# kehanxuuu/vspg-pbrt-v4

Hardware: AMD Instinct MI355X
Metric: Mpaths/sec on 1920x1080 homogeneous fog; relMSE vs CPU ref at equal spp (higher is better)
Workload: dtype f32; 1 GPU; fog-box 1920x1080, guidedvolpathvspg vspguiding=true (primary-ray VSP; App. F options), 1 spp per step per GPU, independent sampler seed 0, maxdepth 5

## Files before the change

### vspg-pbrt-v4_amd/csrc/vspg_capi.hip

```cpp
#include <hip/hip_runtime.h>
#include <dlfcn.h>

#include <cmath>
#include <cstdio>
#include <cstdlib>
#include <cstring>
#include <string>
#include <type_traits>
#include <vector>
#include <algorithm>

#include "vspg_path.h"
#include "vspg_wg_kernel.h"
#include "vspg_guided_wg.h"
#include "vspg_wg3.h"
#include "vspg_trace.h"
#include "vspg_wavefront.h"
#include "vspg_wf_launch.h"
#include "vspg_film_error.h"
#include "vspg_film_resolve.h"
#include "vspg_kernel_choice.h"
#ifdef VSPG_SINGLE_TU
#include "vspg_wf_grid.hip"
#include "vspg_wf_nvdb.hip"
// ... 1807 lines not shown
    return lb;
}
static void build(const VspgScene &sc, const VspgIntegratorParams &prm, DScene *D) {
    DLightSampler *ls = &D->lsamp;
    std::memset(ls, 0, sizeof *ls);
    const int n_all = D->n_lights + D->n_inf;
    for (int i = 0; i < kMaxLights; ++i) ls->bit_trail[i] = 0xffffffffu;
    for (int i = 0; i < VSPG_MAX_QUADS; ++i) ls->light_of_quad[i] = -1;
    for (int i = 0; i < D->n_lights; ++i) ls->light_of_quad[D->light_quads[i]] = i;
    ls->mode = n_all > 1 ? prm.lightsampler : VSPG_LIGHTSAMPLER_UNIFORM;
    lbvh_item_t items[LBVH_MAX_LIGHTS];
    int n_items = 0;
    v3 amin = V3(INFINITY, INFINITY, INFINITY), amax = V3(-INFINITY, -INFINITY, -INFINITY);
    for (int i = 0; i < n_all; ++i) {
        if (i >= D->n_lights) { ls->inf_light[ls->n_inf++] = i; continue; }
        const int qi = D->light_quads[i];
        lightbounds_t lb = quad_light_bounds(D->quads[qi], sc.quads[qi].reverse_orientation);
        if (lb.phi > 0) {
            items[n_items].light = i; items[n_items].lb = lb; n_items++;
            amin = v_min3(amin, lb.bmin); amax = v_max3(amax, lb.bmax);
        }
    }
    if (n_items > 0) { lightbounds_t root; lbvh_build(ls, items, 0, n_items, 0, 0, amin, amax, &root); }
    if (n_all > 0) {
        float pdf[3], power[LBVH_MAX_LIGHTS], acc0 = 0.f;
        for (int i = 0; i < 3; ++i) {
            float up = 0.5f + (float)i / 3;
            if (up > 1) up -= 1;
            float lambda = 538 - 138.888889f * atanhf(0.85691062f - 1.82750197f * up);
            pdf[i] = lambda < 360 || lambda > 830 ? 0.f : 0.0039398042f / sqr(coshf(0.0072f * (lambda - 538)));
        }
        for (int i = 0; i < n_all; ++i) {
            float L[3], k;
            if (i < D->n_lights) {
                const DQuad &q = D->quads[D->light_quads[i]];
                for (int c = 0; c < 3; ++c) L[c] = q.Le[c];
                k = PI_F * (q.two_sided ? 2 : 1) * q.area;
            } else {
                const int j = i - D->n_lights;
                for (int c = 0; c < 3; ++c) L[c] = D->inf_L[j][c];
                k = D->inf_type[j] == VSPG_LIGHT_DISTANT ? PI_F * sqr(D->scene_radius) : 4 * PI_F * PI_F * sqr(D->scene_radius);
            }
            float s = 0.f;
            for (int c = 0; c < 3; ++c) s += pdf[c] != 0 ? (k * L[c]) / pdf[c] : 0.f;
            power[i] = s / 3;
            acc0 += power[i];
        }
        if (acc0 == 0.f) for (int i = 0; i < n_all; ++i) power[i] = 1.f;
        double sum = 0.;
        for (int i = 0; i < n_all; ++i) sum += power[i];
        const float fsum = (float)sum;
        ls->n_alias = n_all;
        struct { float pHat; int index; } under[LBVH_MAX_LIGHTS], over[LBVH_MAX_LIGHTS];
        int nu = 0, no = 0;
        for (int i = 0; i < n_all; ++i) {
            ls->alias_p[i] = power[i] / fsum;
            float pHat = ls->alias_p[i] * n_all;
            if (pHat < 1) { under[nu].pHat = pHat; under[nu].index = i; nu++; } else { over[no].pHat = pHat; over[no].index = i; no++; }
        }
        while (nu > 0 && no > 0) {
            float upH = under[nu - 1].pHat, ovH = over[no - 1].pHat;
            int ui = under[nu - 1].index, oi = over[no - 1].index;
            nu--; no--;
            ls->alias_q[ui] = upH; ls->alias_i[ui] = oi;
            float pExcess = upH + ovH - 1;
            if (pExcess < 1) { under[nu].pHat = pExcess; under[nu].index = oi; nu++; } else { over[no].pHat = pExcess; over[no].index = oi; no++; }
        }
        while (no > 0) { no--; ls->alias_q[over[no].index] = 1; ls->alias_i[over[no].index] = -1; }
        while (nu > 0) { nu--; ls->alias_q[under[nu].index] = 1; ls->alias_i[under[nu].index] = -1; }
    }
}
}

static bool derive_triangle(const float *p9, const float *kd, int id, DTri *T, const int32_t *flags = nullptr);
static int32_t surf_flags_of(int material, int medium_interface) {
    const int b = medium_interface & (VSPG_IFACE_INSIDE | VSPG_IFACE_OUTSIDE);
    const int iface = (b == VSPG_IFACE_INSIDE || b == VSPG_IFACE_OUTSIDE) ? b : 0;
    return (material == VSPG_MATERIAL_INTERFACE ? SURF_INTERFACE : 0) | (iface << SURF_IFACE_SHIFT);
}
static void build_dscene(const VspgScene &sc, const VspgIntegratorParams &prm, const VspgRenderConfig &cfg, DScene *D) {
    using namespace hostmath;
    memset(D, 0, sizeof *D);
    D->n_quads = sc.n_quads;
    for (int i = 0; i < sc.n_quads; ++i) {
        const VspgQuad &in = sc.quads[i];
        DQuad &q = D->quads[i];
        H3 p00 = ld(in.p00), e1 = ld(in.e1), e2 = ld(in.e2);
        H3 p10 = add(p00, e1), p01 = add(p00, e2), p11 = add(p10, e2);
        stv(q.p00, p00); stv(q.p10, p10); stv(q.p01, p01); stv(q.p11, p11); stv(q.e1, e1); stv(q.e2, e2);
        H3 c = crossv(e1, e2);
        q.area = std::sqrt(len2v(c));
        H3 n = normv(c);
        if (in.reverse_orientation) n = H3{-n.x, -n.y, -n.z};
        stv(q.n, n);
        stv(q.dpdu_n, normv(e1));
        const float eps = 0x1p-24f;
        float g6 = (6 * eps) / (1 - 6 * eps);
        H3 s = add(add(absv(p00), absv(p01)), add(absv(p10), absv(p11)));
        stv(q.perr, H3{s.x * g6, s.y * g6, s.z * g6});
        q.inv_l1 = 1.f / len2v(e1);
        q.inv_l2 = 1.f / len2v(e2);
        bool lobes = false, light = false;
        for (int k = 0; k < 3; ++k) {
            float kd = in.Kd[k];
            kd = kd < 0 ? 0 : (kd > 1 ? 1 : kd);
            q.Kd[k] = kd;
            q.Le[k] = in.Le[k];
            lobes = lobes || kd != 0;
            light = light || in.Le[k] != 0;
        }
        q.two_sided = in.two_sided;
        q.is_light = light;
        q.has_lobes = lobes;
        q.flags = surf_flags_of(in.material, in.medium_interface);
        auto single_axis = [](const float *v) {
            int nz = 0, ax = -1;
            for (int k = 0; k < 3; ++k)
                if (v[k] != 0) { nz++; ax = k; }
            return nz == 1 ? ax : -1;
        };
        int an = single_axis(q.n), a1 = single_axis(q.e1), a2 = single_axis(q.e2);
        IsectRec &rec = D->irec[i];
        memset(&rec, 0, sizeof rec);
        if (an >= 0 && a1 >= 0 && a2 >= 0 && an != a1 && an != a2 && a1 != a2 && std::fabs(q.n[an]) == 1.0f) {
            rec.kind = 1;
            rec.axes = an | (a1 << 2) | (a2 << 4);
            rec.f[0] = q.n[an]; rec.f[1] = q.p00[an]; rec.f[2] = q.p00[a1]; rec.f[3] = q.p00[a2];
            rec.f[4] = q.e1[a1]; rec.f[5] = q.e2[a2]; rec.f[6] = q.inv_l1; rec.f[7] = q.inv_l2;
        } else {
            rec.kind = 0;
            for (int k = 0; k < 3; ++k) { rec.f[k] = q.n[k]; rec.f[3 + k] = q.p00[k]; rec.f[6 + k] = q.e1[k]; rec.f[9 + k] = q.e2[k]; }
            rec.f[12] = q.inv_l1; rec.f[13] = q.inv_l2;
        }
        if (light) D->light_quads[D->n_lights++] = i;
    }
    D->n_inf = sc.n_infinite_lights;
    for (int i = 0; i < sc.n_infinite_lights && i < VSPG_MAX_INFINITE_LIGHTS; ++i) {
        D->inf_type[i] = sc.infinite_lights[i].type;
        for (int k = 0; k < 3; ++k) { D->inf_L[i][k] = sc.infinite_lights[i].L[k]; D->inf_w[i][k] = sc.infinite_lights[i].w_light[k]; }
    }
    {
        float lo[3] = {kInf, kInf, kInf}, hi[3] = {-kInf, -kInf, -kInf};
        auto grow = [&](const float *q) { for (int k = 0; k < 3; ++k) { lo[k] = q[k] < lo[k] ? q[k] : lo[k]; hi[k] = q[k] > hi[k] ? q[k] : hi[k]; } };
        for (int i = 0; i < D->n_quads; ++i) { grow(D->quads[i].p00); grow(D->quads[i].p10); grow(D->quads[i].p01); grow(D->quads[i].p11); }
        for (int i = 0; i < sc.n_triangles && sc.tri_p; ++i) {
            DTri T;
            if (derive_triangle(sc.tri_p + 9 * (size_t)i, nullptr, i, &T)) { grow(T.p0); grow(T.p1); grow(T.p2); }
        }
        for (int i = 0; i < sc.n_spheres; ++i) {
            const float *m = sc.spheres[i].render_from_object, rr = sc.spheres[i].radius;
            for (int c = 0; c < 8; ++c) {
                const float x = (c & 1) ? rr : -rr, y = (c & 2) ? rr : -rr, z = (c & 4) ? rr : -rr;
                float q[3];
                for (int k = 0; k < 3; ++k) {
                    volatile float a = m[4 * k] * x;
                    volatile float b = m[4 * k + 1] * y;
                    volatile float c2 = m[4 * k + 2] * z;
                    volatile float sum = a + b;
                    sum = sum + c2;
                    sum = sum + m[4 * k + 3];
                    q[k] = sum;
                }
                grow(q);
            }
        }
        D->scene_radius = 0.f;
        if (lo[0] <= hi[0]) {
            volatile float cx = (lo[0] + hi[0]) / 2, cy = (lo[1] + hi[1]) / 2, cz = (lo[2] + hi[2]) / 2;
            volatile float dx = cx - hi[0], dy = cy - hi[1], dz = cz - hi[2];
            volatile float l2 = dx * dx;
            l2 = l2 + dy * dy;
            l2 = l2 + dz * dz;
            D->scene_radius = std::sqrt(l2);
        }
    }
    D->n_spheres = sc.n_spheres;
    for (int i = 0; i < sc.n_spheres; ++i) {
        const VspgSphere &in = sc.spheres[i];
        DSphere &sp = D->spheres[i];
        for (int k = 0; k < 12; ++k) { sp.m[k] = in.render_from_object[k]; sp.mi[k] = in.object_from_render[k]; }
        sp.radius = in.radius;
        const float *m = in.render_from_object;
        const float minor12 = dop(m[5], m[10], m[6], m[9]), minor02 = dop(m[4], m[10], m[6], m[8]), minor01 = dop(m[4], m[9], m[5], m[8]);
        const bool swaps = std::fmaf(m[2], minor01, dop(m[0], minor12, m[1], minor02)) < 0;
        sp.flip = (in.reverse_orientation ? 1 : 0) ^ (swaps ? 1 : 0);
        auto clamp1 = [](float v) { return v < -1.f ? -1.f : (v > 1.f ? 1.f : v); };
        sp.thetaZMin = std::acos(clamp1(-in.radius / in.radius));
        sp.thetaZMax = std::acos(clamp1(in.radius / in.radius));
        {
            volatile float rad = 3.14159265358979323846f / 180;
            rad = rad * 360.f;
            sp.phiMax = rad;
        }
        bool lobes = false;
        for (int k = 0; k < 3; ++k) {
            float kd = in.Kd[k];
            kd = kd < 0 ? 0 : (kd > 1 ? 1 : kd);
            sp.Kd[k] = kd;
            lobes = lobes || kd != 0;
        }
        sp.has_lobes = lobes;
        sp.flags = surf_flags_of(in.material, in.medium_interface);
    }
    D->camera_in_medium = sc.medium.type != VSPG_MEDIUM_NONE && !sc.camera_outside_medium;
    D->has_boundaries = sc.camera_outside_medium != 0;
    for (int i = 0; i < D->n_quads; ++i) D->has_boundaries |= D->quads[i].flags != 0;
    for (int i = 0; i < D->n_spheres; ++i) D->has_boundaries |= D->spheres[i].flags != 0;
    for (int i = 0; i < sc.n_triangles && sc.tri_flags; ++i)
        D->has_boundaries |= surf_flags_of(sc.tri_flags[i] & VSPG_TRI_INTERFACE, sc.tri_flags[i] >> VSPG_TRI_IFACE_SHIFT) != 0;
    D->cam = sc.camera;
    D->medium_type = sc.medium.type;
    for (int k = 0; k < 3; ++k) {
        D->sigma_a[k] = sc.medium.sigma_a[k];
        D->sigma_s[k] = sc.medium.sigma_s[k];
        {
            volatile float st = D->sigma_s[k] + D->sigma_a[k];
// ... 2049 lines not shown
```

### vspg-pbrt-v4_amd/csrc/vspg_device.h

```cpp
#pragma once
#include <hip/hip_runtime.h>
#include <stdint.h>

#include "../../include/vspg.h"
#include "vspg_arith.h"
#include "vspg_libm.h"

#define VDEV __device__ __forceinline__
#ifdef VSPG_WF_DEBUG
__device__ unsigned int g_dbg_err[8];
#define VSPG_DBG_CHECK(cond, bit) do { if (!(cond)) atomicOr(&g_dbg_err[0], 1u << (bit)); } while (0)
#else
#define VSPG_DBG_CHECK(cond, bit)
#endif
#ifdef VSPG_NOINLINE_LEAVES
#define VLEAF __device__ __attribute__((noinline))
#else
#define VLEAF __device__ __forceinline__
#endif

VSPG_NS_BEGIN

#ifdef VSPG_PROFILE
enum { PS_INTERSECT = 0, PS_HASHRNG, PS_DIST_GUIDED, PS_DIST_PLAIN, PS_SURF_PRE, PS_NEE, PS_NEE_TR, PS_VOL_SAMPLE,
// ... 343 lines not shown
    *cosTheta = ct;
    *sinTheta = safe_sqrt(1 - sqr(ct));
    return 2 * kPi * u1;
}
VDEV V3 hg_post(V3 wo, float g, float sinTheta, float cosTheta, float sinPhi, float cosPhi, float *pdf) {
    g = clampf(g, (float)-.99, (float).99);
    Frame f;
    f.z = wo;
    coordinate_system(wo, &f.x, &f.y);
    V3 local = V3{clampf(sinTheta, -1, 1) * cosPhi, clampf(sinTheta, -1, 1) * sinPhi, clampf(cosTheta, -1, 1)};
    *pdf = henyey_greenstein(cosTheta, g);
    return f.from_local(local);
}
VDEV V3 sample_henyey_greenstein(V3 wo, float g, float u0, float u1, float *pdf) {
    float st, ct;
    float phi = hg_pre(g, u0, u1, &st, &ct);
    return hg_post(wo, g, st, ct, sinf_(phi), cosf_(phi), pdf);
}
VDEV float cos_hemi_pre(float u0, float u1, float *r, bool *degenerate) {
    float ox = 2 * u0 - 1, oy = 2 * u1 - 1;
    *degenerate = (ox == 0 && oy == 0);
    const bool xmajor = __builtin_fabsf(ox) > __builtin_fabsf(oy);
    const float q = (xmajor ? oy : ox) / (xmajor ? ox : oy);
    *r = xmajor ? ox : oy;
    const float t = kPiOver4 * q;
    return xmajor ? t : kPiOver2 - t;
}
VDEV V3 cos_hemi_post(float r, bool degenerate, float sinT, float cosT) {
    float dx = degenerate ? 0.f : r * cosT;
    float dy = degenerate ? 0.f : r * sinT;
    float z = safe_sqrt(1 - sqr(dx) - sqr(dy));
    return V3{dx, dy, z};
}
VDEV V3 sample_cosine_hemisphere(float u0, float u1) {
    float r;
    bool deg;
    float theta = cos_hemi_pre(u0, u1, &r, &deg);
    return cos_hemi_post(r, deg, sinf_(theta), cosf_(theta));
}

struct P3i {
    V3 lo, hi;
    VDEV V3 mid() const { return V3{(lo.x + hi.x) / 2, (lo.y + hi.y) / 2, (lo.z + hi.z) / 2}; }
    VDEV V3 err() const { return V3{(hi.x - lo.x) / 2, (hi.y - lo.y) / 2, (hi.z - lo.z) / 2}; }
};
VDEV P3i p3i_exact(V3 p) { return P3i{p, p}; }
VDEV void interval_ve(float v, float e, float *lo, float *hi) {
    float l = next_float_down(v - e), h = next_float_up(v + e);
    *lo = e == 0 ? v : l;
    *hi = e == 0 ? v : h;
}
VDEV P3i p3i_from_err(V3 p, V3 e) {
    P3i r;
    interval_ve(p.x, e.x, &r.lo.x, &r.hi.x);
    interval_ve(p.y, e.y, &r.lo.y, &r.hi.y);
    interval_ve(p.z, e.z, &r.lo.z, &r.hi.z);
    return r;
}
VDEV float offset_axis(float po, float off) {
    const uint32_t ui = f2b(po), os = f2b(off) & 0x80000000u;
    uint32_t r = ui + ((uint32_t)((int32_t)(ui ^ os) >> 31) | 1u);
    r = (ui << 1) == 0u ? (os | 1u) : r;
    const bool keep = !__builtin_islessgreater(off, 0.f) || (ui ^ os) == 0x7f800000u;
    return b2f(keep ? ui : r);
}
VDEV V3 offset_ray_origin(P3i pi, V3 n, V3 w) {
    float d = dot(vabs(n), pi.err());
    V3 offset = n * d;
    if (dot(w, n) < 0) offset = -offset;
    V3 po = pi.mid() + offset;
    return V3{offset_axis(po.x, offset.x), offset_axis(po.y, offset.y), offset_axis(po.z, offset.z)};
}

#define VSPG_GLOBAL_AS __attribute__((address_space(1)))
struct DQuad {
    float p00[3], p10[3], p01[3], p11[3], e1[3], e2[3];
    float n[3], dpdu_n[3], perr[3];
    float inv_l1, inv_l2, area;
    float Kd[3], Le[3];
    int32_t two_sided, is_light, has_lobes;
    int32_t flags;
};
enum { SURF_INTERFACE = 1, SURF_IFACE_SHIFT = 1 };
struct IsectRec {
    float f[14];
    int32_t kind;
    int32_t axes;
};
struct DField {
    int32_t n_nodes, n_regions;
    const VspgKdNode *nodes;
    const VspgFieldRegion *regions;
    const float *aux;
    const float4 *lobes;
};
constexpr int kMaxLights = VSPG_MAX_QUADS + VSPG_MAX_INFINITE_LIGHTS;
struct DLightNode {
    float bmin[3], bmax[3], w[3];
    float phi, cosTheta_o, cosTheta_e;
    int32_t twoSided;
    uint32_t child_or_light;
    int32_t is_leaf;
};
struct DLightSampler {
    int32_t mode;
    int32_t n_nodes, n_inf, n_alias;
    DLightNode nodes[2 * kMaxLights];
    int32_t inf_light[VSPG_MAX_INFINITE_LIGHTS];
    uint32_t bit_trail[kMaxLights];
    float alias_p[kMaxLights], alias_q[kMaxLights];
    int32_t alias_i[kMaxLights];
    int32_t light_of_quad[VSPG_MAX_QUADS];
};
struct DTri {
    float p0[3], nx;
    float p1[3], ny;
    float p2[3], nz;
    float dpdu_n[3];
    int32_t id;
    float Kd[3];
    int32_t flags;
};
struct DSphere {
    float m[12], mi[12];
    float radius, thetaZMin, thetaZMax, phiMax;
    float Kd[3];
    int32_t flip, has_lobes, flags;
};
struct DBvh4Node {
    float lox[4], loy[4], loz[4], hix[4], hiy[4], hiz[4];
    int32_t child[4];
    int32_t pad[4];
};
static_assert(sizeof(DBvh4Node) == 128, "one node = eight 16-byte loads");
constexpr int32_t kBvhAbsent = (int32_t)0x80000000;
constexpr int kBvhStack = 48;
struct PixelWindow {
    int32_t x0, y0, x1, y1;
};
__host__ __device__ __forceinline__ int win_tile_x0(const PixelWindow &w) { return w.x0 >> 3; }
__host__ __device__ __forceinline__ int win_tile_y0(const PixelWindow &w) { return w.y0 >> 3; }
__host__ __device__ __forceinline__ int win_tiles_x(const PixelWindow &w) { return ((w.x1 + 7) >> 3) - (w.x0 >> 3); }
__host__ __device__ __forceinline__ int win_tiles_y(const PixelWindow &w) { return ((w.y1 + 7) >> 3) - (w.y0 >> 3); }
__host__ __device__ __forceinline__ bool win_has(const PixelWindow &w, int px, int py) { return px >= w.x0 && px < w.x1 && py >= w.y0 && py < w.y1; }
struct DScene {
    int32_t n_quads, n_lights;
    int32_t n_tris, n_bvh_nodes;
    int32_t n_spheres, has_boundaries, camera_in_medium, pad_b;
    VspgCamera cam;
    int32_t medium_type;
    float sigma_a[3], sigma_s[3], Le[3], g;
    float sigma_t[3], sigma_n_raw[3];
    VspgIntegratorParams prm;
    int32_t xres, yres, seed, shard_index, shard_count;
    DSphere spheres[VSPG_MAX_SPHERES];
    const DTri *tris;
    const DBvh4Node *bvh;
    int32_t n_inf;
    int32_t inf_type[VSPG_MAX_INFINITE_LIGHTS];
    float inf_L[VSPG_MAX_INFINITE_LIGHTS][3], inf_w[VSPG_MAX_INFINITE_LIGHTS][3];
    float scene_radius;
    DField field[2];
    IsectRec irec[VSPG_MAX_QUADS];
    int32_t light_quads[VSPG_MAX_QUADS];
    DQuad quads[VSPG_MAX_QUADS];
    int32_t nx, ny, nz;
    float bounds_min[3], bounds_max[3];
    const float *density;
    const float *majorant;
    const int32_t *brick_index;
    const float4 *octets;
    int32_t bnx, bny, bnz;
    int32_t has_xform;
    float minv[12];
    int32_t index_min[3];
    float inv_voxel[3], grid_origin[3], density_offset;
    const float *le_scale;
    int32_t le_nx, le_ny, le_nz;
    const float *temperature;
    float temperature_offset, temperature_scale, nvdb_le_scale;
    float *tr_rgb;
    int32_t *tr_spp;
    int32_t tr_calc, tr_load;
    const float *contrib;
    int32_t contrib_ready;
    DLightSampler lsamp;
};
#ifdef VSPG_NO_BOUNDARIES
template <int BND> VDEV bool has_bnd(const DScene &) { return false; }
#else
template <int BND> VDEV bool has_bnd(const DScene &S) {
    if constexpr (BND >= 0) return BND != 0;
    else return S.has_boundaries != 0;
}
#endif
enum { VSP_READY = 1, VSP_NO_FEED = 2 };

__shared__ DQuad s_scene_quads[VSPG_MAX_QUADS];
__shared__ int32_t s_scene_light_quads[VSPG_MAX_QUADS];
enum { MED_SIGMA_A = 0, MED_SIGMA_S = 3, MED_LE = 6, MED_G = 9, MED_SIGMA_T = 10, MED_SIGMA_N_RAW = 13, MED_COUNT = 16 };
__shared__ float s_scene_medium[MED_COUNT];
VDEV void stage_scene_lds(const DScene &S) {
    vspg_libm::stage_logf_tab_lds();
    vspg_libm::stage_log_tab_lds();
    const uint32_t *src = reinterpret_cast<const uint32_t *>(S.quads);
    uint32_t *dst = reinterpret_cast<uint32_t *>(s_scene_quads);
    const int n = S.n_quads * (int)(sizeof(DQuad) / 4);
    for (int i = threadIdx.x; i < n; i += blockDim.x) dst[i] = src[i];
    if (threadIdx.x < VSPG_MAX_QUADS) s_scene_light_quads[threadIdx.x] = S.light_quads[threadIdx.x];
    if (threadIdx.x < MED_COUNT) {
        const int k = threadIdx.x;
        s_scene_medium[k] = k < 3 ? S.sigma_a[k] : k < 6 ? S.sigma_s[k - 3] : k < 9 ? S.Le[k - 6] : k == 9 ? S.g
                            : k < 13 ? S.sigma_t[k - 10] : S.sigma_n_raw[k - 13];
    }
}
VDEV const DQuad &quad_at(int i) { return s_scene_quads[i]; }
VDEV const DQuad &light_quad_at(int lightIndex) { return s_scene_quads[s_scene_light_quads[lightIndex]]; }

struct Isect {
    bool hit;
    float t;
    int quad;
    V3 p, n;
};
VDEV bool is_tri(int prim) { return prim <= -2; }
VDEV int tri_of(int prim) { return -2 - prim; }
constexpr int kSpherePrim = 32;
static_assert(VSPG_MAX_QUADS <= kSpherePrim, "rectangle indices lie below the first sphere primitive");
VDEV bool is_sphere(int prim) { return prim >= kSpherePrim; }
VDEV int sphere_of(int prim) { return prim - kSpherePrim; }

VDEV bool beyond(float num, float denom, float tMax) {
    return __builtin_fabsf(num) > tMax * __builtin_fabsf(denom) * 1.000001f;
}
VDEV float comp(V3 v, int axis) { return axis == 0 ? v.x : (axis == 1 ? v.y : v.z); }
VDEV bool rect_hit_uv(const IsectRec &r, V3 o, V3 d, float tMax, float *tHit, float *uHit, float *vHit) {
    float num, denom, u, v, t;
    if (r.kind == 1) {
        const int a = r.axes & 3, ua = (r.axes >> 2) & 3, va = (r.axes >> 4) & 3;
        denom = r.f[0] * comp(d, a);
        num = r.f[0] * (r.f[1] - comp(o, a));
        bool cand = (num > 0 && denom > 0) || (num < 0 && denom < 0);
        if (!cand) return false;
        if (beyond(num, denom, tMax)) return false;
        t = num / denom;
        if (!(t > 0) || !(t < tMax)) return false;
        float pu = comp(o, ua) + comp(d, ua) * t, pv = comp(o, va) + comp(d, va) * t;
        u = ((pu - r.f[2]) * r.f[4]) * r.f[6];
        v = ((pv - r.f[3]) * r.f[5]) * r.f[7];
    } else {
        V3 n = V3{r.f[0], r.f[1], r.f[2]}, p00 = V3{r.f[3], r.f[4], r.f[5]};
        denom = dot(n, d);
        num = dot(n, p00 - o);
        bool cand = (num > 0 && denom > 0) || (num < 0 && denom < 0);
        if (!cand) return false;
        if (beyond(num, denom, tMax)) return false;
        t = num / denom;
        if (!(t > 0) || !(t < tMax)) return false;
        V3 p = o + d * t;
        V3 rel = p - p00;
        u = dot(rel, V3{r.f[6], r.f[7], r.f[8]}) * r.f[12];
        v = dot(rel, V3{r.f[9], r.f[10], r.f[11]}) * r.f[13];
    }
    if (u < 0 || u > 1 || v < 0 || v > 1) return false;
    *tHit = t;
    *uHit = u;
    *vHit = v;
    return true;
}
VDEV bool quad_hit_uv(const DQuad &q, V3 o, V3 d, float tMax, float *tHit, float *uHit, float *vHit) {
    V3 n = ld3(q.n), p00 = ld3(q.p00);
    float denom = dot(n, d);
    float num = dot(n, p00 - o);
    bool cand = (num > 0 && denom > 0) || (num < 0 && denom < 0);
    if (!cand) return false;
    float t = num / denom;
    if (!(t > 0) || !(t < tMax)) return false;
    V3 p = o + d * t;
    V3 rel = p - p00;
    float u = dot(rel, ld3(q.e1)) * q.inv_l1;
    float v = dot(rel, ld3(q.e2)) * q.inv_l2;
    if (u < 0 || u > 1 || v < 0 || v > 1) return false;
    *tHit = t;
    *uHit = u;
    *vHit = v;
    return true;
}
VDEV V3 quad_point(const DQuad &q, float u, float v) { return ld3(q.p00) + (ld3(q.e1) * u + ld3(q.e2) * v); }
VDEV bool quad_intersect(const DQuad &q, V3 o, V3 d, float tMax, float *tHit, V3 *pHit) {
    float u, v;
    if (!quad_hit_uv(q, o, d, tMax, tHit, &u, &v)) return false;
    *pHit = quad_point(q, u, v);
    return true;
}
struct TriHit { float t, b0, b1, b2; };
VDEV V3 permute3(V3 v, int kx, int ky, int kz) { return V3{comp(v, kx), comp(v, ky), comp(v, kz)}; }
VDEV float max3abs(float a, float b, float c) { return fmax_(fmax_(__builtin_fabsf(a), __builtin_fabsf(b)), __builtin_fabsf(c)); }
struct TriRay {
    int kx, ky, kz;
    float Sx, Sy, Sz;
};
VDEV TriRay tri_ray(V3 d) {
    TriRay R;
    const V3 ad = vabs(d);
    R.kz = (ad.x > ad.y) ? ((ad.x > ad.z) ? 0 : 2) : ((ad.y > ad.z) ? 1 : 2);
    R.kx = R.kz + 1; if (R.kx == 3) R.kx = 0;
    R.ky = R.kx + 1; if (R.ky == 3) R.ky = 0;
    const V3 dp = permute3(d, R.kx, R.ky, R.kz);
    R.Sx = -dp.x / dp.z; R.Sy = -dp.y / dp.z; R.Sz = 1 / dp.z;
    return R;
}
VDEV bool tri_intersect(V3 o, const TriRay &R, float tMax, V3 p0, V3 p1, V3 p2, TriHit *hit) {
    V3 p0t = p0 - o, p1t = p1 - o, p2t = p2 - o;
    const int kx = R.kx, ky = R.ky, kz = R.kz;
    p0t = permute3(p0t, kx, ky, kz); p1t = permute3(p1t, kx, ky, kz); p2t = permute3(p2t, kx, ky, kz);
    const float Sx = R.Sx, Sy = R.Sy, Sz = R.Sz;
    p0t.x += Sx * p0t.z; p0t.y += Sy * p0t.z;
    p1t.x += Sx * p1t.z; p1t.y += Sy * p1t.z;
    p2t.x += Sx * p2t.z; p2t.y += Sy * p2t.z;
    float e0 = diff_of_products(p1t.x, p2t.y, p1t.y, p2t.x);
    float e1 = diff_of_products(p2t.x, p0t.y, p2t.y, p0t.x);
    float e2 = diff_of_products(p0t.x, p1t.y, p0t.y, p1t.x);
    if (e0 == 0.0f || e1 == 0.0f || e2 == 0.0f) {
        const double p2txp1ty = (double)p2t.x * (double)p1t.y, p2typ1tx = (double)p2t.y * (double)p1t.x;
        e0 = (float)(p2typ1tx - p2txp1ty);
        const double p0txp2ty = (double)p0t.x * (double)p2t.y, p0typ2tx = (double)p0t.y * (double)p2t.x;
        e1 = (float)(p0typ2tx - p0txp2ty);
        const double p1txp0ty = (double)p1t.x * (double)p0t.y, p1typ0tx = (double)p1t.y * (double)p0t.x;
        e2 = (float)(p1typ0tx - p1txp0ty);
    }
    if ((e0 < 0 || e1 < 0 || e2 < 0) && (e0 > 0 || e1 > 0 || e2 > 0)) return false;
    const float det = e0 + e1 + e2;
    if (det == 0) return false;
    p0t.z *= Sz; p1t.z *= Sz; p2t.z *= Sz;
    const float tScaled = e0 * p0t.z + e1 * p1t.z + e2 * p2t.z;
    if (det < 0 && (tScaled >= 0 || tScaled < tMax * det)) return false;
    else if (det > 0 && (tScaled <= 0 || tScaled > tMax * det)) return false;
    const float invDet = 1 / det;
    const float b0 = e0 * invDet, b1 = e1 * invDet, b2 = e2 * invDet;
    const float t = tScaled * invDet;
    constexpr float g2 = (2 * kMachineEps) / (1 - 2 * kMachineEps), g3 = (3 * kMachineEps) / (1 - 3 * kMachineEps),
                    g5 = (5 * kMachineEps) / (1 - 5 * kMachineEps);
    const float maxZt = max3abs(p0t.z, p1t.z, p2t.z);
    const float deltaZ = g3 * maxZt;
    const float maxXt = max3abs(p0t.x, p1t.x, p2t.x), maxYt = max3abs(p0t.y, p1t.y, p2t.y);
    const float deltaX = g5 * (maxXt + maxZt), deltaY = g5 * (maxYt + maxZt);
    const float deltaE = 2 * (g2 * maxXt * maxYt + deltaY * maxXt + deltaX * maxYt);
    const float maxE = max3abs(e0, e1, e2);
    const float deltaT = 3 * (g3 * maxE * maxZt + deltaE * maxZt + deltaZ * maxE) * __builtin_fabsf(invDet);
    if (t <= deltaT) return false;
    hit->t = t; hit->b0 = b0; hit->b1 = b1; hit->b2 = b2;
// ... 121 lines not shown
    for (int k = 0; k < 3; ++k) {
        const float *row = S.mi + 4 * k;
        const float v = (row[0] * ro.x + row[1] * ro.y) + (row[2] * ro.z + row[3]);
        const float e = g3 * (__builtin_fabsf(row[0] * ro.x) + __builtin_fabsf(row[1] * ro.y) + __builtin_fabsf(row[2] * ro.z) + __builtin_fabsf(row[3]));
        oi[k] = ivl_from_err(v, e);
        const float ev = g3 * (__builtin_fabsf(row[0] * rd.x) + __builtin_fabsf(row[1] * rd.y) + __builtin_fabsf(row[2] * rd.z));
        const float vv = row[0] * rd.x + row[1] * rd.y + row[2] * rd.z;
        di[k] = ivl_from_err(vv, ev);
    }
    const Ivl a = ivl_add(ivl_add(ivl_sqr(di[0]), ivl_sqr(di[1])), ivl_sqr(di[2]));
    const Ivl b = ivl_fmul(2.f, ivl_add(ivl_add(ivl_mul(di[0], oi[0]), ivl_mul(di[1], oi[1])), ivl_mul(di[2], oi[2])));
    const Ivl c = ivl_sub(ivl_add(ivl_add(ivl_sqr(oi[0]), ivl_sqr(oi[1])), ivl_sqr(oi[2])), ivl_sqr(ivl_x(S.radius)));
    const Ivl f = ivl_div(b, ivl_fmul(2.f, a));
    const Ivl v0 = ivl_sub(oi[0], ivl_mul(f, di[0])), v1 = ivl_sub(oi[1], ivl_mul(f, di[1])), v2 = ivl_sub(oi[2], ivl_mul(f, di[2]));
    const Ivl length = ivl_sqrt(ivl_add(ivl_add(ivl_sqr(v0), ivl_sqr(v1)), ivl_sqr(v2)));
    const Ivl discrim = ivl_mul(ivl_mul(ivl_fmul(4.f, a), ivl_add(ivl_x(S.radius), length)), ivl_sub(ivl_x(S.radius), length));
    if (discrim.lo < 0) return false;
    const Ivl rootDiscrim = ivl_sqrt(discrim);
    Ivl q;
    if (ivl_mid(b) < 0) q = ivl_fmul(-.5f, ivl_sub(b, rootDiscrim));
    else q = ivl_fmul(-.5f, ivl_add(b, rootDiscrim));
    Ivl t0 = ivl_div(q, a), t1 = ivl_div(c, q);
    if (t0.lo > t1.lo) { const Ivl t = t0; t0 = t1; t1 = t; }
    if (t0.hi > tMax || t1.lo <= 0) return false;
    Ivl tShapeHit = t0;
    if (tShapeHit.lo <= 0) {
        tShapeHit = t1;
        if (tShapeHit.hi > tMax) return false;
    }
    const float ts = ivl_mid(tShapeHit);
    V3 pHit = V3{ivl_mid(oi[0]) + ts * ivl_mid(di[0]), ivl_mid(oi[1]) + ts * ivl_mid(di[1]), ivl_mid(oi[2]) + ts * ivl_mid(di[2])};
    const float sc = S.radius / len(pHit);
    pHit = V3{pHit.x * sc, pHit.y * sc, pHit.z * sc};
    if (pHit.x == 0 && pHit.y == 0) pHit.x = 1e-5f * S.radius;
    *tHit = ts;
    *pObj = pHit;
    return true;
}
struct SphereSurf {
    P3i pi;
    V3 n, dpdu_n;
};
template <bool WITH_DPDU = true>
VDEV SphereSurf sphere_interaction(const DSphere &S, V3 pHit) {
    SphereSurf r;
    const float cosTheta = pHit.z / S.radius;
    const float zRadius = __builtin_sqrtf(sqr(pHit.x) + sqr(pHit.y));
    const float cosPhi = pHit.x / zRadius, sinPhi = pHit.y / zRadius;
    const V3 dpdu = V3{-S.phiMax * pHit.y, S.phiMax * pHit.x, 0.f};
    const float sinTheta = safe_sqrt(1 - sqr(cosTheta));
    const float dth = S.thetaZMax - S.thetaZMin;
    const V3 dpdv = V3{dth * (pHit.z * cosPhi), dth * (pHit.z * sinPhi), dth * (-S.radius * sinTheta)};
    V3 no = normalize(cross(dpdu, dpdv));
    if (S.flip) no = -no;
    constexpr float g5 = (5 * kMachineEps) / (1 - 5 * kMachineEps), g3 = (3 * kMachineEps) / (1 - 3 * kMachineEps);
    const Ivl px = ivl_from_err(pHit.x, g5 * __builtin_fabsf(pHit.x)), py = ivl_from_err(pHit.y, g5 * __builtin_fabsf(pHit.y)),
              pz = ivl_from_err(pHit.z, g5 * __builtin_fabsf(pHit.z));
    const float x = ivl_mid(px), y = ivl_mid(py), z = ivl_mid(pz);
    const float ex = (px.hi - px.lo) / 2, ey = (py.hi - py.lo) / 2, ez = (pz.hi - pz.lo) / 2;
    const bool exact = (px.hi - px.lo) == 0 && (py.hi - py.lo) == 0 && (pz.hi - pz.lo) == 0;
    float pv[3], pe[3];
#pragma unroll
    for (int k = 0; k < 3; ++k) {
        const float *row = S.m + 4 * k;
        pv[k] = (row[0] * x + row[1] * y) + (row[2] * z + row[3]);
        const float ea = g3 * (__builtin_fabsf(row[0] * x) + __builtin_fabsf(row[1] * y) + __builtin_fabsf(row[2] * z) + __builtin_fabsf(row[3]));
        pe[k] = exact ? ea : (g3 + 1) * (__builtin_fabsf(row[0]) * ex + __builtin_fabsf(row[1]) * ey + __builtin_fabsf(row[2]) * ez) + ea;
    }
    r.pi = p3i_from_err(V3{pv[0], pv[1], pv[2]}, V3{pe[0], pe[1], pe[2]});
    const float *mi = S.mi;
    r.n = normalize(V3{mi[0] * no.x + mi[4] * no.y + mi[8] * no.z, mi[1] * no.x + mi[5] * no.y + mi[9] * no.z, mi[2] * no.x + mi[6] * no.y + mi[10] * no.z});
    if (WITH_DPDU) {
        const float *m = S.m;
        r.dpdu_n = normalize(V3{m[0] * dpdu.x + m[1] * dpdu.y + m[2] * dpdu.z, m[4] * dpdu.x + m[5] * dpdu.y + m[6] * dpdu.z, m[8] * dpdu.x + m[9] * dpdu.y + m[10] * dpdu.z});
    } else {
        r.dpdu_n = mk(0, 0, 0);
    }
    return r;
}

template <bool FULL = true>
VLEAF Isect scene_intersect(const DScene &S, V3 o, V3 d, float tMax) {
    Isect best;
    best.hit = false;
    best.t = tMax;
    best.quad = 0;
    float bu = 0, bv = 0;
    for (int i = 0; i < S.n_quads; ++i) {
        float t, u, v;
        if (rect_hit_uv(S.irec[i], o, d, best.t, &t, &u, &v)) {
            best.hit = true;
            best.t = t;
            best.quad = i;
            bu = u;
            bv = v;
        }
    }
    const DQuad &q = quad_at(best.quad);
    best.p = quad_point(q, bu, bv);
    best.n = ld3(q.n);
    if (FULL && S.n_tris > 0) {
        int tp = 0;
        TriHit h;
        if (bvh_closest(S, o, d, best.t, &tp, &h)) {
            const DTri &T = S.tris[tp];
            best.hit = true;
            best.t = h.t;
            best.quad = -2 - tp;
            best.p = V3{h.b0, h.b1, h.b2};
            best.n = V3{T.nx, T.ny, T.nz};
        }
    }
    if (FULL && S.n_spheres > 0) {
        for (int i = 0; i < S.n_spheres; ++i) {
            float t;
            V3 pObj;
            if (sphere_intersect(S.spheres[i], o, d, tMax, &t, &pObj) && t < best.t) {
                best.hit = true;
                best.t = t;
                best.quad = kSpherePrim + i;
                best.p = pObj;
                best.n = sphere_interaction<false>(S.spheres[i], pObj).n;
            }
        }
    }
    return best;
}
template <bool FULL = true>
VLEAF bool scene_intersect_any(const DScene &S, V3 o, V3 d, float tMax) {
    bool any = false;
    for (int i = 0; i < S.n_quads; ++i) {
        float t, u, v;
        any = any || rect_hit_uv(S.irec[i], o, d, tMax, &t, &u, &v);
    }
    if (FULL && S.n_tris > 0 && !any) any = bvh_any(S, o, d, tMax);
    if (FULL && S.n_spheres > 0 && !any) {
        for (int i = 0; i < S.n_spheres; ++i) {
            float t;
            V3 pObj;
            any = any || sphere_intersect(S.spheres[i], o, d, tMax, &t, &pObj);
        }
    }
    return any;
}
VDEV int surf_flags(const DScene &S, int prim) {
    if (is_tri(prim)) return S.tris[tri_of(prim)].flags;
    if (is_sphere(prim)) return S.spheres[sphere_of(prim)].flags;
    return quad_at(prim).flags;
}
VDEV P3i tri_pi(const DTri &T, V3 b) {
    const V3 p0 = ld3(T.p0), p1 = ld3(T.p1), p2 = ld3(T.p2);
    const V3 p = p0 * b.x + p1 * b.y + p2 * b.z;
    const V3 s = vabs(p0 * b.x) + vabs(p1 * b.y) + vabs(p2 * b.z);
    constexpr float g7 = (7 * kMachineEps) / (1 - 7 * kMachineEps);
    return p3i_from_err(p, V3{g7 * s.x, g7 * s.y, g7 * s.z});
}
template <bool FULL = true>
VDEV P3i surf_pi(const DScene &S, int prim, V3 p) {
    if (FULL && is_sphere(prim)) return sphere_interaction<false>(S.spheres[sphere_of(prim)], p).pi;
    if (FULL && is_tri(prim)) return tri_pi(S.tris[tri_of(prim)], p);
    return p3i_from_err(p, ld3(quad_at(prim).perr));
}
VDEV float dot_vn(V3 v, V3 n) {
    const float cd = n.z * v.z;
    const float sop = __builtin_fmaf(n.y, v.y, cd);
    const float err = __builtin_fmaf(n.z, v.z, -cd);
    return __builtin_fmaf(n.x, v.x, sop + err);
}
VDEV bool get_medium(int flags, V3 n, V3 w, bool medium) {
    const int iface = flags >> SURF_IFACE_SHIFT;
    if (iface) return dot_vn(w, n) > 0 ? (iface & VSPG_IFACE_OUTSIDE) != 0 : (iface & VSPG_IFACE_INSIDE) != 0;
    return medium;
}

struct MediumProps {
    Spec sigma_a, sigma_s, Le;
    float g;
    Spec sigma_t;
    float bb_temp = 0.f, bb_scale = 0.f;
};
struct MajSeg {
    float tMin, tMax;
    Spec sigma_maj;
};
template <int GREY, bool NULLZERO = false, bool SIMPLE = false>
struct HomogeneousMediumT {
    static constexpr int kGrey = GREY;
    static constexpr bool kNullZero = NULLZERO;
    static constexpr bool kSimpleScene = SIMPLE;
    static constexpr int kBnd = -1;
    static VDEV Spec m3(int o) {
        if constexpr (GREY) {
            const float x = s_scene_medium[o];
            return Spec{x, x, x};
        }
        return Spec{s_scene_medium[o], s_scene_medium[o + 1], s_scene_medium[o + 2]};
    }
    struct Iter {
        MajSeg seg;
        bool called;
        VDEV bool next(MajSeg *s) {
            if (called) return false;
            called = true;
            *s = seg;
            return true;
        }
    };
    VDEV Iter sample_ray(V3, V3, float tMax) const { return Iter{MajSeg{0, tMax, m3(MED_SIGMA_T)}, false}; }
    VDEV MediumProps sample_point(V3) const {
        return MediumProps{m3(MED_SIGMA_A), m3(MED_SIGMA_S), m3(MED_LE), s_scene_medium[MED_G], m3(MED_SIGMA_T)};
    }
    VDEV Spec sigma_n(const MediumProps &, Spec) const { return clamp_zero(m3(MED_SIGMA_N_RAW)); }
    VDEV bool is_homogeneous() const { return true; }
    static constexpr bool kSingleSegment = true;
    static constexpr bool kAlwaysRealCollision = true;
    static constexpr bool kEmit = false;
};
// ... 586 lines not shown
```

Before: 3616 Mpaths/s.

## Rotate ray into quad axis frame incrementally to avoid per-component selects

Axis-aligned quad records now store a relative rotation step from the previous quad's axis frame, plus a uv-swap flag. The intersection loop rotates the ray origin and direction cumulatively with register swaps, so the aligned test reads fixed components instead of using runtime-indexed comp() selects. This is meant to cut the select/ALU cost of the per-quad rectangle test in the hot intersection loop. In exchange it adds a small swap loop per quad and a loop-carried dependence, and correctness relies on the records being built in order.

```diff
diff --git a/vspg-pbrt-v4_amd/csrc/vspg_capi.hip b/vspg-pbrt-v4_amd/csrc/vspg_capi.hip
--- a/vspg-pbrt-v4_amd/csrc/vspg_capi.hip
+++ b/vspg-pbrt-v4_amd/csrc/vspg_capi.hip
@@ -1913,6 +1913,7 @@
     using namespace hostmath;
     memset(D, 0, sizeof *D);
     D->n_quads = sc.n_quads;
+    int frame = 0;
     for (int i = 0; i < sc.n_quads; ++i) {
         const VspgQuad &in = sc.quads[i];
         DQuad &q = D->quads[i];
@@ -1944,25 +1945,7 @@
         q.is_light = light;
         q.has_lobes = lobes;
         q.flags = surf_flags_of(in.material, in.medium_interface);
-        auto single_axis = [](const float *v) {
-            int nz = 0, ax = -1;
-            for (int k = 0; k < 3; ++k)
-                if (v[k] != 0) { nz++; ax = k; }
-            return nz == 1 ? ax : -1;
-        };
-        int an = single_axis(q.n), a1 = single_axis(q.e1), a2 = single_axis(q.e2);
-        IsectRec &rec = D->irec[i];
-        memset(&rec, 0, sizeof rec);
-        if (an >= 0 && a1 >= 0 && a2 >= 0 && an != a1 && an != a2 && a1 != a2 && std::fabs(q.n[an]) == 1.0f) {
-            rec.kind = 1;
-            rec.axes = an | (a1 << 2) | (a2 << 4);
-            rec.f[0] = q.n[an]; rec.f[1] = q.p00[an]; rec.f[2] = q.p00[a1]; rec.f[3] = q.p00[a2];
-            rec.f[4] = q.e1[a1]; rec.f[5] = q.e2[a2]; rec.f[6] = q.inv_l1; rec.f[7] = q.inv_l2;
-        } else {
-            rec.kind = 0;
-            for (int k = 0; k < 3; ++k) { rec.f[k] = q.n[k]; rec.f[3 + k] = q.p00[k]; rec.f[6 + k] = q.e1[k]; rec.f[9 + k] = q.e2[k]; }
-            rec.f[12] = q.inv_l1; rec.f[13] = q.inv_l2;
-        }
+        frame = isect_rec_build(&D->irec[i], q.n, q.p00, q.e1, q.e2, q.inv_l1, q.inv_l2, frame);
         if (light) D->light_quads[D->n_lights++] = i;
     }
     D->n_inf = sc.n_infinite_lights;
diff --git a/vspg-pbrt-v4_amd/csrc/vspg_device.h b/vspg-pbrt-v4_amd/csrc/vspg_device.h
--- a/vspg-pbrt-v4_amd/csrc/vspg_device.h
+++ b/vspg-pbrt-v4_amd/csrc/vspg_device.h
@@ -449,11 +449,43 @@
     int32_t flags;
 };
 enum { SURF_INTERFACE = 1, SURF_IFACE_SHIFT = 1 };
+enum { kIsectStepsMask = 3, kIsectUvSwapped = 4, kIsectAxisAligned = 8, kIsectAxisShift = 4 };
 struct IsectRec {
     float f[14];
     int32_t kind;
     int32_t axes;
 };
+inline int isect_rec_build(IsectRec *rec, const float *n, const float *p00, const float *e1, const float *e2, float inv_l1, float inv_l2, int cur) {
+    int ax[3];
+    const float *vec[3] = {n, e1, e2};
+    for (int j = 0; j < 3; ++j) {
+        int nz = 0;
+        ax[j] = -1;
+        for (int k = 0; k < 3; ++k)
+            if (vec[j][k] != 0) { nz++; ax[j] = k; }
+        if (nz != 1) ax[j] = -1;
+    }
+    const int an = ax[0], a1 = ax[1], a2 = ax[2];
+    for (int k = 0; k < 14; ++k) rec->f[k] = 0;
+    int frame = 0;
+    bool swapped = false;
+    if (an >= 0 && an <= 2 && a1 >= 0 && a2 >= 0 && an != a1 && an != a2 && a1 != a2 && (n[an] == 1.0f || n[an] == -1.0f)) {
+        swapped = a1 != (an + 1) % 3;
+        const int au = swapped ? a2 : a1, av = swapped ? a1 : a2;
+        frame = an;
+        rec->kind = 1;
+        rec->f[0] = n[an]; rec->f[1] = p00[an]; rec->f[2] = p00[au]; rec->f[3] = p00[av];
+        rec->f[4] = swapped ? e2[a2] : e1[a1]; rec->f[5] = swapped ? e1[a1] : e2[a2];
+        rec->f[6] = swapped ? inv_l2 : inv_l1; rec->f[7] = swapped ? inv_l1 : inv_l2;
+    } else {
+        rec->kind = 0;
+        for (int k = 0; k < 3; ++k) { rec->f[k] = n[k]; rec->f[3 + k] = p00[k]; rec->f[6 + k] = e1[k]; rec->f[9 + k] = e2[k]; }
+        rec->f[12] = inv_l1; rec->f[13] = inv_l2;
+    }
+    if (cur < 0 || cur > 2) cur = 0;
+    rec->axes = ((frame - cur + 3) % 3) | (swapped ? kIsectUvSwapped : 0) | (rec->kind == 1 ? kIsectAxisAligned : 0) | (frame << kIsectAxisShift);
+    return frame;
+}
 struct DField {
     int32_t n_nodes, n_regions;
     const VspgKdNode *nodes;
@@ -601,18 +633,26 @@
     return __builtin_fabsf(num) > tMax * __builtin_fabsf(denom) * 1.000001f;
 }
 VDEV float comp(V3 v, int axis) { return axis == 0 ? v.x : (axis == 1 ? v.y : v.z); }
+VDEV void swap_regs(float &a, float &b) { asm("v_swap_b32 %0, %1" : "+v"(a), "+v"(b)); }
+VDEV void rect_frame(V3 &o, V3 &d, int steps) {
+#pragma nounroll
+    for (int k = steps & kIsectStepsMask; k > 0; --k) {
+        swap_regs(o.x, o.y);
+        swap_regs(o.y, o.z);
+        swap_regs(d.x, d.y);
+        swap_regs(d.y, d.z);
+    }
+}
 VDEV bool rect_hit_uv(const IsectRec &r, V3 o, V3 d, float tMax, float *tHit, float *uHit, float *vHit) {
     float num, denom, u, v, t;
-    if (r.kind == 1) {
-        const int a = r.axes & 3, ua = (r.axes >> 2) & 3, va = (r.axes >> 4) & 3;
-        denom = r.f[0] * comp(d, a);
-        num = r.f[0] * (r.f[1] - comp(o, a));
-        bool cand = (num > 0 && denom > 0) || (num < 0 && denom < 0);
-        if (!cand) return false;
+    if (r.axes & kIsectAxisAligned) {
+        denom = d.x;
+        num = r.f[1] - o.x;
+        if ((int32_t)(__builtin_bit_cast(uint32_t, num) ^ __builtin_bit_cast(uint32_t, denom)) < 0) return false;
         if (beyond(num, denom, tMax)) return false;
         t = num / denom;
         if (!(t > 0) || !(t < tMax)) return false;
-        float pu = comp(o, ua) + comp(d, ua) * t, pv = comp(o, va) + comp(d, va) * t;
+        float pu = o.y + d.y * t, pv = o.z + d.z * t;
         u = ((pu - r.f[2]) * r.f[4]) * r.f[6];
         v = ((pv - r.f[3]) * r.f[5]) * r.f[7];
     } else {
@@ -634,6 +674,41 @@
     *uHit = u;
     *vHit = v;
     return true;
+}
+VDEV bool rects_closest(const IsectRec *recs, int n, V3 o, V3 d, float tMax, float *tBest, int *iBest, float *uBest, float *vBest) {
+    bool hit = false;
+    float bt = tMax, bu = 0, bv = 0;
+    int bi = 0;
+    V3 fo = o, fd = d;
+    for (int i = 0; i < n; ++i) {
+        const IsectRec &r = recs[i];
+        float t, u, v;
+        rect_frame(fo, fd, r.axes);
+        if (rect_hit_uv(r, fo, fd, bt, &t, &u, &v)) {
+            const bool swapped = (r.axes & kIsectUvSwapped) != 0;
+            hit = true;
+            bt = t;
+            bi = i;
+            bu = swapped ? v : u;
+            bv = swapped ? u : v;
+        }
+    }
+    *tBest = bt;
+    *iBest = bi;
+    *uBest = bu;
+    *vBest = bv;
+    return hit;
+}
+VDEV bool rects_any(const IsectRec *recs, int n, V3 o, V3 d, float tMax) {
+    bool any = false;
+    V3 fo = o, fd = d;
+    for (int i = 0; i < n; ++i) {
+        const IsectRec &r = recs[i];
+        float t, u, v;
+        rect_frame(fo, fd, r.axes);
+        any = any || rect_hit_uv(r, fo, fd, tMax, &t, &u, &v);
+    }
+    return any;
 }
 VDEV bool quad_hit_uv(const DQuad &q, V3 o, V3 d, float tMax, float *tHit, float *uHit, float *vHit) {
     V3 n = ld3(q.n), p00 = ld3(q.p00);
@@ -921,20 +996,8 @@
 template <bool FULL = true>
 VLEAF Isect scene_intersect(const DScene &S, V3 o, V3 d, float tMax) {
     Isect best;
-    best.hit = false;
-    best.t = tMax;
-    best.quad = 0;
-    float bu = 0, bv = 0;
-    for (int i = 0; i < S.n_quads; ++i) {
-        float t, u, v;
-        if (rect_hit_uv(S.irec[i], o, d, best.t, &t, &u, &v)) {
-            best.hit = true;
-            best.t = t;
-            best.quad = i;
-            bu = u;
-            bv = v;
-        }
-    }
+    float bu, bv;
+    best.hit = rects_closest(S.irec, S.n_quads, o, d, tMax, &best.t, &best.quad, &bu, &bv);
     const DQuad &q = quad_at(best.quad);
     best.p = quad_point(q, bu, bv);
     best.n = ld3(q.n);
@@ -967,11 +1030,7 @@
 }
 template <bool FULL = true>
 VLEAF bool scene_intersect_any(const DScene &S, V3 o, V3 d, float tMax) {
-    bool any = false;
-    for (int i = 0; i < S.n_quads; ++i) {
-        float t, u, v;
-        any = any || rect_hit_uv(S.irec[i], o, d, tMax, &t, &u, &v);
-    }
+    bool any = rects_any(S.irec, S.n_quads, o, d, tMax);
     if (FULL && S.n_tris > 0 && !any) any = bvh_any(S, o, d, tMax);
     if (FULL && S.n_spheres > 0 && !any) {
         for (int i = 0; i < S.n_spheres; ++i) {
```

Result: faster. 3812 Mpaths/s (median of 6 runs) (+5.4%).
